# NickQrumpton/lattice-gaussian-mcmc

Measured on AMD Instinct MI355X. Metric: Klein samples/sec at n=512 NTRU (IMHK proposals, d=1024), higher is better.
Workload: dtype f64

## Files before the change

### lattice-gaussian-mcmc_amd/csrc/lgs_capi.hip

```cpp
#include <hip/hip_runtime.h>

#include <algorithm>
#include <cmath>
#include <cstdarg>
#include <cstdio>
#include <cstdlib>
#include <climits>
#include <cstring>
#include <string>
#include <vector>

#include "../../include/lgs.h"
#include "lgs_kernels.h"
#include "lgs_szc_host.h"

namespace {

thread_local std::string g_err;

int fail(int code, const char* fmt, ...) {
    char buf[512];
    va_list ap;
    va_start(ap, fmt);
    vsnprintf(buf, sizeof(buf), fmt, ap);
// ... 109 lines not shown
    bool has_rd = false, oz_off = false;
    DevBuf H16, F0;
    DevBuf ZNZ;
    DevBuf CLIVE;
    DevBuf VNP;
    DevBuf LAGP;
    struct {
        const void* Z = nullptr;
        int64_t lanes = 0, cols = 0;
        const unsigned int* clive = nullptr;
        int64_t clive_ld = 0;
    } hist;
    DevBuf Bd;
    DevBuf kchunk, koff;
    bool bz_mom_ok = false;
    DevBuf MP;
    DevBuf etab;
    DevBuf etab2;
    DevBuf szc;
    bool libm_samplez = false;
    bool has_Bi8 = false;
    int64_t bd_rows = 0, bd_cols = 0;
    std::vector<BzCall> pending_i8;
    bool i8_dev_replay = false;
    DevBuf Z, LW, V, sel, fsel, cnt, ccnt, flags, stage_a, stage_b, stage_c, stage_d, stage_e,
        stage_f, stage_g, stage_h, stage_i, vs;
    int64_t max_props = 1 << 18;
    bool max_props_user = false;
    bool no_pipe = false, no_look = false, no_qskip = false, no_cu_split = false;
    int zint = 2;
    bool timing = false;
    double t_ms[7] = {0, 0, 0, 0, 0, 0, 0};
    int64_t t_n[7] = {0, 0, 0, 0, 0, 0, 0};
    DevBuf dg_x, dg_y, dg_out, dg_a, dg_b, dg_c, dg_t;
    DevBuf DQ, DBIT;
    bool has_q = false, has_binv = false;
    std::vector<Timer> pending;
    std::vector<hipEvent_t> pool;
    unsigned int* fw_host = nullptr;
    hipEvent_t fw_ev = nullptr;
    struct BlockSet {
        DevBuf Z, LW, H16, ZNZ, CLIVE, flags;
        hipEvent_t ev_free = nullptr;
        bool free_recorded = false;
    } bset[3];
    int bset_next = 0;
    int nsets = 2;
    bool kstream_sets_fixed = false;
    hipStream_t kstream = nullptr;
    hipStream_t kstream_full = nullptr, kstream_split = nullptr;
    int cu_split = 0;
    int kstream_cus = 0;
    int split_cus = 0;
    hipEvent_t kt0 = nullptr, kt1 = nullptr;
    bool kt_pending = false;
    double kt_bz_ms = 0.0;
    hipEvent_t ev_klein = nullptr;
    struct Spec {
        bool valid = false;
        uint64_t seed = 0, chain0 = 0, step0 = 0;
        int64_t nc = 0, Tb = 0, ldzb = 0;
        int zb = 0, j = 0;
        bool wl = false, exact = false, oz = false;
        decltype(hist) h;
        hipEvent_t ev = nullptr;
    } spec;
};

// ... 46 lines not shown
struct SetSwap {
    lgs_ctx* c = nullptr;
    int j = -1;
    bool flags_in = false, store_in = false;
    void swap_flags() {
        swap_buf(c->flags, c->bset[j].flags);
        flags_in = !flags_in;
    }
    void swap_store() {
        auto& s = c->bset[j];
        swap_buf(c->Z, s.Z);
        swap_buf(c->LW, s.LW);
        swap_buf(c->H16, s.H16);
        swap_buf(c->ZNZ, s.ZNZ);
        swap_buf(c->CLIVE, s.CLIVE);
        store_in = !store_in;
    }
    void restore() {
        if (j < 0) return;
        if (store_in) swap_store();
        if (flags_in) swap_flags();
    }
    bool record = true;
    void release() {
        if (j < 0) return;
        restore();
        if (record) {
            (void)hipEventRecord(c->bset[j].ev_free, c->stream);
            c->bset[j].free_recorded = true;
        }
        j = -1;
    }
    ~SetSwap() { release(); }
};

constexpr double kBzStoreBytesPerMs = 4.6e9;
static int split_decide(lgs_ctx* c) {
    if (c->cu_split != 0 || !c->kt_pending || hipEventQuery(c->kt1) != hipSuccess) return LGS_OK;
    c->kt_pending = false;
    float ms = 0.f;
    if (hipEventElapsedTime(&ms, c->kt0, c->kt1) != hipSuccess || !(ms > 0.f)) return LGS_OK;
    const int ncu = c->split_cus * 8 / 7;
    const double cost = (double)ms * (double)(ncu - c->split_cus) / (double)c->split_cus;
    if (c->kt_bz_ms > cost) {
        HIP_TRY(hipStreamSynchronize(c->kstream_full));
        c->kstream = c->kstream_split;
        c->kstream_cus = c->split_cus;
        c->cu_split = 1;
    } else {
        c->cu_split = 2;
    }
    return LGS_OK;
}

int spec_discard(lgs_ctx* c) {
    if (!c->spec.valid) return LGS_OK;
    c->spec.valid = false;
    HIP_TRY(hipStreamSynchronize(c->kstream));
    HIP_TRY(hipMemset(c->bset[c->spec.j].flags.p, 0, 4 * lgs::kFlagWords));
    size_t keep = 0;
    for (auto& t : c->pending) {
        if (t.spec) {
            c->pool.push_back(t.a);
            c->pool.push_back(t.b);
        } else {
            c->pending[keep++] = t;
        }
    }
    c->pending.resize(keep);
    return LGS_OK;
}

int settle_bz(lgs_ctx* c, const unsigned int* f0_known = nullptr) {
    if (!f0_known) HIP_TRY(hipStreamSynchronize(c->stream));
    if (c->pending_i8.empty() && !c->i8_dev_replay) return LGS_OK;
    {
        unsigned int f0 = 0;
        if (f0_known)
            f0 = *f0_known;
        else
            HIP_TRY(hipMemcpy(&f0, c->flags.p, sizeof(f0), hipMemcpyDeviceToHost));
// ... 23 lines not shown
        c->z1cap = 2.0 * std::max(z1, c->z1seen);
        c->z1seen = z1;
    }
}

void fold_timers(lgs_ctx* c) {
    size_t keep = 0;
    for (auto& t : c->pending) {
        if (t.spec || hipEventQuery(t.b) != hipSuccess) {
            c->pending[keep++] = t;
            continue;
        }
        float ms = 0;
        if (hipEventElapsedTime(&ms, t.a, t.b) == hipSuccess) {
            c->t_ms[t.kernel] += ms;
            c->t_n[t.kernel] += 1;
        }
        c->pool.push_back(t.a);
        c->pool.push_back(t.b);
    }
    c->pending.resize(keep);
}

int finish(lgs_ctx* c, const unsigned int* fw_known = nullptr, bool clear_all = false) {
    int rc0 = settle_bz(c, fw_known);
    if (rc0) return rc0;
    fold_timers(c);
    unsigned int fw[lgs::kFlagWords] = {};
    if (fw_known)
        memcpy(fw, fw_known, sizeof(fw));
    else
        HIP_TRY(hipMemcpy(fw, c->flags.p, sizeof(fw), hipMemcpyDeviceToHost));
    const unsigned int f = fw[0];
    c->resolved_seen = 0;
    if (fw[1] || fw[2] || fw[3])
        fold_counters(c, fw);
    c->n_accept_resolved += fw[lgs::kFlagWordAcceptResolved];
    c->n_wl_mismatch += fw[lgs::kFlagWordWLMismatch];
    c->n_qskip += fw[lgs::kFlagWordQSkip];
    bool any = false;
    for (int k = 1; k < lgs::kFlagWords; ++k) any |= fw[k] != 0;
    if (clear_all)
        HIP_TRY(hipMemsetAsync(c->flags.p, 0, lgs::kFlagWords * sizeof(unsigned int), c->stream));
    else if (any)
        HIP_TRY(hipMemsetAsync((unsigned int*)c->flags.p + 1, 0, (lgs::kFlagWords - 1) * sizeof(unsigned int),
                               c->stream));
    if (f & lgs::kFlagNonFinite)
        return fail(LGS_ERR_NONFINITE, "non-finite conditional mean (reference raises ValueError)");
    if (f & lgs::kFlagOverflow)
        return fail(LGS_ERR_OVERFLOW, "coefficient |z| >= 2^31: rerun with LGS_Z64");
    return LGS_OK;
}

int finish_or_redo(lgs_ctx* c, bool oz_used, int& zb, bool& redo, bool early = false) {
    redo = false;
    unsigned int fw[lgs::kFlagWords];
    if (early) {
        HIP_TRY(hipEventSynchronize(c->fw_ev));
        memcpy(fw, c->fw_host, sizeof(fw));
    } else {
        HIP_TRY(hipStreamSynchronize(c->stream));
        HIP_TRY(hipMemcpy(fw, c->flags.p, sizeof(fw), hipMemcpyDeviceToHost));
    }
    if (!(fw[0] & lgs::kAbortMask)) return finish(c, fw, early);
    c->pending_i8.clear();
    c->i8_dev_replay = false;
    for (auto& t : c->pending) {
        c->pool.push_back(t.a);
        c->pool.push_back(t.b);
    }
    c->pending.clear();
    c->n_fallback += 1;
    c->n_resolved += fw[kFlagWordCheckpoint];
    if (fw[0] & lgs::kFlagOverflow16) {
        if (zb == 2) c->zint = 4;
        if (oz_used) c->oz_off = true;
    }
    if (fw[0] & lgs::kFlagCarry16) c->zint = 4;
    if (zb == 2) zb = c->zint;
    HIP_TRY(hipMemsetAsync(c->flags.p, 0, 4 * lgs::kFlagWords, c->stream));
    redo = true;
    return LGS_OK;
}

int reset_flags(lgs_ctx* c) {
    int rc = c->flags.reserve(4 * lgs::kFlagWords);
    if (rc) return rc;
    c->resolved_seen = 0;
    HIP_TRY(hipMemsetAsync(c->flags.p, 0, 4 * lgs::kFlagWords, c->stream));
    return LGS_OK;
}

lgs::KleinArgs base_args(lgs_ctx* c, uint64_t seed) {
    lgs::KleinArgs a{};
    const double* co = c->coord.as<double>();
    const int64_t d = c->d;
    a.d = (int)d;
    a.precision = c->precision;
    a.linear_probs = (c->basis_flags & LGS_BASIS_LINEAR_PROBS) ? 1 : 0;
    a.cp = co;
    a.rii = co + d;
    a.sig = co + 2 * d;
    a.sig_ref = co + 3 * d;
// ... 101 lines not shown
    if (zb == 2) {
        c->zint = 4;
        zb = 4;
    }
    if (oz) c->oz_off = true;
    c->hist.Z = nullptr;
    rc = run_klein(c, a, exact, wl, zb, Z, oz);
    if (oz_out) *oz_out = oz;
    return rc;
}

int run_bz_fp64(lgs_ctx* c, const BzCall& b) {
    Scope s(c, 1);
    HIP_TRY(lgs::launch::bz(b.Z, b.zb, b.ldz, b.sel, c->BT.as<double>(), (int)c->d, b.n, b.V, c->d, b.rb,
                            b.rstride, b.roff, c->stream));
    if (b.VN) HIP_TRY(lgs::launch::vnorm2_rows(b.V, (int)c->d, b.vn_n, b.rb, b.rstride, b.roff, b.VN, c->stream));
    return LGS_OK;
}

int run_bz(lgs_ctx* c, const void* Z, int zb, int64_t ldz, int64_t n, double* V,
           int64_t rb = 0, int64_t rstride = 0, int64_t roff = 0, const int64_t* sel = nullptr,
           bool after_klein = false, const unsigned int* abort = nullptr, double* VN = nullptr,
           int64_t vn_n = -1, bool device_replay = false, unsigned long long* MP = nullptr,
           int64_t mp_ld = 0, unsigned int* MPL = nullptr) {
    if (!c->has_B) return fail(LGS_ERR_STATE, "lattice points need B (lgs_set_basis B != NULL)");
    if (vn_n < 0 || vn_n > n) vn_n = n;
    if (vn_n == 0) VN = nullptr;
    BzCall b{Z, zb, ldz, n, V, rb > 0 ? rb : n, rstride, roff, sel, VN, vn_n};
    static const bool force64 = hook_is("LGS_BZ_FP64", 1);
    if (!c->has_Bi8 || force64) {
        Scope s(c, 1);
        HIP_TRY(lgs::launch::bz(b.Z, b.zb, b.ldz, b.sel, c->BT.as<double>(), (int)c->d, b.n, b.V, c->d, b.rb,
                                b.rstride, b.roff, c->stream, abort));
        if (VN) HIP_TRY(lgs::launch::vnorm2_rows(b.V, (int)c->d, vn_n, b.rb, b.rstride, b.roff, VN, c->stream));
        return LGS_OK;
    }
    Scope s(c, 1);
    const int8_t* hi = c->Bd.as<int8_t>();
    const int8_t* lo = hi + (size_t)c->bd_rows * c->bd_cols;
    static const int diag_bz = hook("LGS_DIAG_BZ") ? atoi(hook("LGS_DIAG_BZ")) : 0;
    if (diag_bz & 1) VN = nullptr;
    if (diag_bz & 2) sel = nullptr;
    double* VNP = nullptr;
    if (VN) {
        const int rc = c->VNP.reserve((size_t)2 * ((c->d + lgs::kBzBN - 1) / lgs::kBzBN) * vn_n * 8);
        if (rc) return rc;
        VNP = c->VNP.as<double>();
    }
    HIP_TRY(lgs::launch::bz_i8(Z, zb, ldz, sel, c->kchunk.as<int>(), c->koff.as<int>(), hi, lo,
                               (int)c->bd_cols, (int)c->d, n, V, c->d, b.rb,
                               b.rstride, b.roff, c->flags.as<unsigned int>(),
                               after_klein && c->hist.Z == Z && Z ? c->H16.as<int16_t>() : nullptr, c->hist.lanes,
                               c->hist.cols, c->stream, abort, c->ZNZ.as<uint8_t>(),
                               after_klein && c->hist.Z == Z && Z ? c->hist.clive : nullptr, c->hist.clive_ld,
                               VNP, vn_n, MP, mp_ld, MPL));
    if (VN) HIP_TRY(lgs::launch::vnorm2_reduce(VNP, (int)c->d, vn_n, b.rb, b.rstride, b.roff, VN, c->stream, abort));
    if (device_replay) {
        c->i8_dev_replay = true;
        const unsigned int* need = c->flags.as<unsigned int>();
        HIP_TRY(lgs::launch::bz(b.Z, b.zb, b.ldz, b.sel, c->BT.as<double>(), (int)c->d, b.n, b.V, c->d, b.rb,
                                b.rstride, b.roff, c->stream, abort, need));
        if (VN)
            HIP_TRY(lgs::launch::vnorm2_rows(b.V, (int)c->d, vn_n, b.rb, b.rstride, b.roff, VN, c->stream, abort,
                                             need));
        return LGS_OK;
    }
    c->pending_i8.push_back(b);
    return LGS_OK;
}

int lookahead(lgs_ctx* c, int j, uint64_t seed, uint64_t first_chain, uint64_t step0, int64_t nc, int64_t tb,
              bool carry, int zb, bool exact, bool wl) {
    const auto hist = c->hist;
    SetSwap sw;
    sw.c = c;
    sw.j = j;
    sw.record = false;
    sw.swap_flags();
    sw.swap_store();
    const int64_t ldz = nc * tb + (carry ? nc : 0);
    lgs::KleinArgs a = base_args(c, seed);
    a.counter_mode = 1;
    a.chain0 = (uint32_t)first_chain;
    a.step0 = (uint32_t)step0;
    a.nt = tb;
    a.n = nc * tb;
    a.ldz = ldz;
    a.LW = c->LW.as<double>();
    auto& bs = c->bset[j];
    if (bs.free_recorded) HIP_TRY(hipStreamWaitEvent(c->kstream, bs.ev_free, 0));
// ... 796 lines not shown
        }
        if ((rc = spec_discard(c))) return rc;
        for (int si = 0; si < c->nsets; ++si) {
            auto& s = c->bset[si];
            s.Z.release();
            s.LW.release();
            s.H16.release();
            s.ZNZ.release();
            s.CLIVE.release();
        }
        c->Z.release();
        c->LW.release();
        c->cnt.release();
        c->LWE.release();
        c->H16.release();
        c->ZNZ.release();
        c->CLIVE.release();
        c->hist = decltype(c->hist){};
        maxp = std::max<int64_t>(nc * thin, maxp / 2);
        c->max_props = maxp;
        c->max_props_user = true;
    }
    const bool no_look = c->no_look || hook_is("LGS_NO_LOOKAHEAD", 1);
    bool spec_hit = false;
    if (c->spec.valid) {
        const int64_t tb0 = std::min<int64_t>(T, n_steps);
        const auto& sp = c->spec;
        spec_hit = pipe && sp.seed == seed && sp.chain0 == first_chain && sp.step0 == first_step && sp.nc == nc &&
                   sp.Tb == tb0 && sp.ldzb == nc * tb0 + (carry ? nc : 0) && sp.zb == zb && sp.wl == wl &&
                   sp.exact == exact && sp.j == c->bset_next;
        if (!spec_hit && (rc = spec_discard(c))) return rc;
    }

    void* zs = z_state;
    double* lws = logw_state;
    int32_t* init = state_init;
    int64_t* acc = accepts;
    if (!dev) {
        if ((rc = c->stage_a.reserve((size_t)nc * d * ob)) || (rc = c->stage_b.reserve((size_t)nc * 8)) ||
            (rc = c->stage_c.reserve((size_t)nc * 4)) || (rc = c->stage_d.reserve((size_t)nc * 8)))
            return rc;
        zs = c->stage_a.p;
        lws = c->stage_b.as<double>();
        init = c->stage_c.as<int32_t>();
        acc = c->stage_d.as<int64_t>();
        HIP_TRY(hipMemcpyAsync(zs, z_state, (size_t)nc * d * ob, hipMemcpyHostToDevice, c->stream));
        HIP_TRY(hipMemcpyAsync(lws, logw_state, nc * 8, hipMemcpyHostToDevice, c->stream));
        HIP_TRY(hipMemcpyAsync(init, state_init, nc * 4, hipMemcpyHostToDevice, c->stream));
        HIP_TRY(hipMemcpyAsync(acc, accepts, nc * 8, hipMemcpyHostToDevice, c->stream));
    }
    double* lwk = logw_samples;
    uint8_t* accs = accepted;
    if (!dev && (logw_samples || accepted)) {
        if ((rc = c->stage_h.reserve((size_t)std::max<int64_t>(nc * n_keep, 1) * 8)) ||
            (rc = c->stage_i.reserve((size_t)std::max<int64_t>(nc * n_steps, 1))))
            return rc;
        lwk = logw_samples ? c->stage_h.as<double>() : nullptr;
        accs = accepted ? (uint8_t*)c->stage_i.p : nullptr;
    }
    unsigned long long* mom = nullptr;
    if (moments) {
        if (dev) {
            mom = (unsigned long long*)moments;
        } else {
            if ((rc = c->stage_e.reserve((size_t)2 * d * 8))) return rc;
            mom = c->stage_e.as<unsigned long long>();
            HIP_TRY(hipMemcpyAsync(mom, moments, (size_t)2 * d * 8, hipMemcpyHostToDevice, c->stream));
        }
    }
    unsigned int* fl = c->flags.as<unsigned int>();

    const uint64_t next_step = first_step + (uint64_t)n_steps;
    bool look_done = false;
    static const bool look_late = !hook_is("LGS_LOOKAHEAD_EARLY", 1);
    for (int64_t t0 = 0; t0 < n_steps || t0 == 0;) {
        bool oz_used = false;
        SetSwap sw;
        if (pipe) {
            sw.c = c;
            sw.j = c->bset_next;
            sw.swap_flags();
            fl = c->flags.as<unsigned int>();
        }
        if (t0 == 0) {
            HIP_TRY(lgs::launch::uninit_scan(init, nc, fl + kFlagWordUninit, c->stream));
            lgs::KleinArgs a = base_args(c, seed);
            a.counter_mode = 1;
            a.chain0 = (uint32_t)first_chain;
            a.step0 = 0;
            a.nt = 1;
            a.n = nc;
            a.ldz = nc;
            a.LW = c->LW.as<double>();
            if (certw) a.emax = c->EMAX.as<unsigned long long>();
            a.gate = fl + kFlagWordUninit;
            bool oz0 = false;
            if ((rc = run_klein_store(c, a, exact, wl, zb, c->Z.p, true, &oz0))) return rc;
            oz_used |= oz0;
            HIP_TRY(lgs::launch::init_apply(c->Z.p, zb, init, nc, (int)d, c->LW.as<double>(), zs, ob, cm, lws,
// ... 4 lines not shown
            if ((rc = finish_or_redo(c, oz_used, zb, redo))) return rc;
            if (redo) continue;
            break;
        }
        const int64_t Tb = std::min<int64_t>(T, n_steps - t0);
        const int64_t npb = nc * Tb;
        const int64_t first_keep = t0 / thin;
        const int64_t kb = std::min<int64_t>(Tb / thin, n_keep - first_keep);
        if (pipe) sw.swap_store();
        lgs::KleinArgs a = base_args(c, seed);
        a.counter_mode = 1;
        a.chain0 = (uint32_t)first_chain;
        a.step0 = (uint32_t)(first_step + (uint64_t)t0);
        const int64_t ldzb = npb + (carry ? nc : 0);
        a.nt = Tb;
        a.n = npb;
        a.ldz = ldzb;
        a.LW = c->LW.as<double>();
        if (certw) {
            a.LWE = c->LWE.as<double>();
            a.emax = c->EMAX.as<unsigned long long>();
        }
        bool ozb = false;
        if (pipe && spec_hit && t0 == 0) {
            spec_hit = false;
            c->spec.valid = false;
            for (auto& t : c->pending) t.spec = false;
            ozb = c->spec.oz;
            c->hist = c->spec.h;
            HIP_TRY(hipStreamWaitEvent(c->stream, c->spec.ev, 0));
        } else if (pipe) {
            auto& bs = c->bset[sw.j];
            if (bs.free_recorded) HIP_TRY(hipStreamWaitEvent(c->kstream, bs.ev_free, 0));
            const hipStream_t cs = c->stream;
            const bool timed = c->cu_split == 0 && !c->kt_pending;
            if (timed) HIP_TRY(hipEventRecord(c->kt0, c->kstream));
            c->stream = c->kstream;
            rc = run_klein_store(c, a, exact, wl, zb, c->Z.p, true, &ozb);
            c->stream = cs;
            if (rc) return rc;
            if (timed) {
                HIP_TRY(hipEventRecord(c->kt1, c->kstream));
                c->kt_pending = true;
                c->kt_bz_ms = carry ? (double)nc * (double)kb * 8.0 * (double)d / kBzStoreBytesPerMs : 0.0;
            }
            HIP_TRY(hipEventRecord(c->ev_klein, c->kstream));
            HIP_TRY(hipStreamWaitEvent(c->stream, c->ev_klein, 0));
        } else if ((rc = run_klein_store(c, a, exact, wl, zb, c->Z.p, true, &ozb))) {
            return rc;
        }
        if (pipe && !no_look && !look_late && !look_done && t0 + T >= n_steps &&
            next_step + (uint64_t)n_steps <= (1ull << 32)) {
            look_done = true;
            if ((rc = lookahead(c, (sw.j + 1) % c->nsets, seed, first_chain, next_step, nc, std::min<int64_t>(T, n_steps), carry,
                                zb, exact, wl)))
                return rc;
        }
        oz_used |= ozb;
        if (carry && kb > 0)
            HIP_TRY(lgs::launch::carry_cols(zs, ob, cm, nc, (int)d, c->Z.p, zb, ldzb, npb, c->stream, fl));
        if (early) {
            HIP_TRY(hipMemcpyAsync(c->fw_host, fl, 4 * lgs::kFlagWords, hipMemcpyDeviceToHost, c->stream));
            HIP_TRY(hipEventRecord(c->fw_ev, c->stream));
        }
        if (moments) HIP_TRY(hipMemsetAsync(c->cnt.p, 0, (size_t)npb * 4, c->stream));
        lgs::AcceptArgs aa{};
        aa.nc = nc;
        aa.T = Tb;
        aa.thin = thin;
        aa.n_keep = std::max<int64_t>(kb, 1);
        aa.seed = seed;
        aa.chain0 = (uint32_t)first_chain;
        aa.step0 = a.step0;
        aa.LW = c->LW.as<double>();
        aa.lw_state = lws;
        aa.accepts = acc;
        aa.sel = (z_samples || v_samples || zk_samples) && kb > 0 ? c->sel.as<int64_t>() : nullptr;
        aa.final_sel = c->fsel.as<int64_t>();
        aa.carry_col = carry ? npb : -1;
// ... 21 lines not shown
            aa.bscale = bs ? std::max(1.0, atof(bs)) : 1.0;
        }
        {
            Scope s(c, 2);
            HIP_TRY(lgs::launch::accept(aa, a, c->stream));
        }
        static const bool no_bz_mom = hook_is("LGS_NO_BZ_MOMENTS", 1);
        static const bool bz_f64 = hook_is("LGS_BZ_FP64", 1);
        const bool bz_mom = moments && v_samples && early && thin == 1 && kb == Tb && kb > 0 && zb == 2 &&
                            c->has_Bi8 && c->bz_mom_ok && !bz_f64 && c->hist.Z == c->Z.p && c->hist.Z &&
                            c->hist.clive != nullptr && lgs::launch::bz_moments_supported() &&
                            d % 16 == 0 && d <= lgs::kOzMaxD && npb < ((int64_t)1 << 32) && !no_bz_mom;
        const bool fuse_final = !bz_mom && moments && !((z_samples || zk_samples) && kb > 0 && !carry) &&
                                npb < ((int64_t)1 << 32);
        if (moments && !bz_mom) {
            Scope s(c, 3);
            HIP_TRY(lgs::launch::moments_carry(zs, ob, cm, nc, (int)d, c->ccnt.as<int32_t>(), mom, c->stream, fl));
            const bool zflags = c->hist.Z == c->Z.p && c->hist.Z != nullptr;
            HIP_TRY(lgs::launch::moments_final(c->Z.p, zb, ldzb, c->cnt.as<int32_t>(), npb, Tb,
                                               fuse_final ? c->fsel.as<int64_t>() : nullptr, (int)d, mom, zs,
                                               ob, cm, nc, c->stream, fl, zflags ? c->ZNZ.as<uint8_t>() : nullptr,
                                               c->hist.lanes, (int)((16 - d % 16) % 16)));
        }
        if ((z_samples || v_samples || zk_samples) && kb > 0) {
            const int64_t nq = nc * kb;
            if (v_samples) {
                const bool dev_replay = early || (lag && lag->lag_v_sums && vnorm2_samples);
                const int64_t ntiles = (nq + 63) / 64, mp_ld = c->bd_cols;
                const int64_t ngw = (d + 2047) / 2048;
                unsigned int* mpl = nullptr;
                if (bz_mom) {
                    if ((rc = c->MP.reserve((size_t)ntiles * (mp_ld * 8 + ngw * 4)))) return rc;
                    mpl = (unsigned int*)(c->MP.as<unsigned long long>() + (size_t)ntiles * mp_ld);
                }
                if ((rc = run_bz(c, c->Z.p, zb, ldzb, nq, v_samples, kb, n_keep, first_keep,
                                 c->sel.as<int64_t>(), true, fl, vnorm2_samples, fn_chains * kb, dev_replay,
                                 bz_mom ? c->MP.as<unsigned long long>() : nullptr, mp_ld, mpl)))
                    return rc;
                if (bz_mom) {
                    Scope s(c, 3);
                    HIP_TRY(lgs::launch::bz_moments_reduce(c->MP.as<unsigned long long>(), mpl, ntiles, mp_ld,
                                                           (int)d, mom, fl, c->stream, fl));
                    HIP_TRY(lgs::launch::moments_carry(zs, ob, cm, nc, (int)d, c->ccnt.as<int32_t>(), mom,
                                                       c->stream, fl, fl));
                    HIP_TRY(lgs::launch::moments_final(c->Z.p, zb, ldzb, c->cnt.as<int32_t>(), npb, Tb, nullptr,
                                                       (int)d, mom, zs, ob, cm, nc, c->stream, fl,
                                                       c->ZNZ.as<uint8_t>(), c->hist.lanes, 0, fl));
                }
            }
            if (zk_samples)
                HIP_TRY(lgs::launch::coord_gather(c->Z.p, zb, ldzb, c->sel.as<int64_t>(), fn_chains * kb, kb, zs, ob, cm, nc,
                                                  (int)d, (int)zk_index, zk_samples, kb, n_keep, first_keep,
                                                  c->stream, fl));
            if (lag) {
                const int L = (int)lag->lag_L;
                if ((rc = c->LAGP.reserve((size_t)(L + 2) * fn_chains * 8))) return rc;
                if (lag->lag_z_sums)
                    HIP_TRY(lgs::launch::lag_update(zk_samples + first_keep, 0, n_keep, fn_chains, kb, L, 1.0,
                                                    lag->lag_z_ring, lag->lag_z_sums, c->LAGP.p, c->stream, fl));
                if (lag->lag_v_sums)
                    HIP_TRY(lgs::launch::lag_update(vnorm2_samples + first_keep, 1, n_keep, fn_chains, kb, L,
                                                    lag->lag_v_scale, lag->lag_v_ring, lag->lag_v_sums, c->LAGP.p,
                                                    c->stream, fl));
            }
            if (z_samples) {
                if ((rc = c->stage_f.reserve((size_t)nq * d * ob))) return rc;
                HIP_TRY(lgs::launch::gather_z(c->Z.p, zb, ldzb, c->sel.as<int64_t>(), nq, kb, zs, ob, cm,
                                              nc, (int)d, c->stage_f.p, 1, c->stream, fl));
                if ((rc = c->stage_g.reserve((size_t)nq * d * ob))) return rc;
                HIP_TRY(lgs::launch::transpose_out(c->stage_f.p, ob, nq, nq, (int)d, c->stage_g.p,
                                                   ob, c->stream));
                HIP_TRY(hipMemcpy2DAsync((char*)z_samples + (size_t)first_keep * d * ob,
                                         (size_t)n_keep * d * ob, c->stage_g.p, (size_t)kb * d * ob,
                                         (size_t)kb * d * ob, nc, kind_of(dev, true), c->stream));
            }
        }
        if (bz_mom)
            HIP_TRY(lgs::launch::final_h16(c->H16.as<int16_t>(), c->hist.lanes, c->fsel.as<int64_t>(), nc, (int)d,
                                           zs, ob, cm, c->stream, fl));
        else if (!fuse_final)
            HIP_TRY(lgs::launch::gather_z(c->Z.p, zb, ldzb, c->fsel.as<int64_t>(), nc, 1, zs, ob, cm, nc,
                                          (int)d, zs, cm, c->stream, fl));
        bool redo = false;
        if ((rc = finish_or_redo(c, oz_used, zb, redo, early))) return rc;
        if (pipe) {
            sw.release();
            fl = c->flags.as<unsigned int>();
            if (!redo) c->bset_next = (c->bset_next + 1) % c->nsets;
        }
        if (redo) continue;
        t0 += T;
    }
    if (pipe && (rc = split_decide(c))) return rc;
    if (pipe && !no_look && look_late && next_step + (uint64_t)n_steps <= (1ull << 32))
        if ((rc = lookahead(c, c->bset_next, seed, first_chain, next_step, nc, std::min<int64_t>(T, n_steps), carry, zb,
                            exact, wl)))
            return rc;
    if (!dev) {
        HIP_TRY(hipMemcpyAsync(z_state, zs, (size_t)nc * d * ob, hipMemcpyDeviceToHost, c->stream));
        HIP_TRY(hipMemcpyAsync(logw_state, lws, nc * 8, hipMemcpyDeviceToHost, c->stream));
        HIP_TRY(hipMemcpyAsync(state_init, init, nc * 4, hipMemcpyDeviceToHost, c->stream));
        HIP_TRY(hipMemcpyAsync(accepts, acc, nc * 8, hipMemcpyDeviceToHost, c->stream));
        if (moments)
            HIP_TRY(hipMemcpyAsync(moments, mom, (size_t)2 * d * 8, hipMemcpyDeviceToHost, c->stream));
        if (logw_samples && n_keep > 0)
            HIP_TRY(hipMemcpyAsync(logw_samples, lwk, (size_t)nc * n_keep * 8, hipMemcpyDeviceToHost, c->stream));
        if (accepted && n_steps > 0)
            HIP_TRY(hipMemcpyAsync(accepted, accs, (size_t)nc * n_steps, hipMemcpyDeviceToHost, c->stream));
        HIP_TRY(hipStreamSynchronize(c->stream));
    }
    return LGS_OK;
}

int lgs_sample_z(lgs_ctx* c, int64_t n, const double* mu, const double* sigma, const double* u,
                 int32_t precision, int64_t* z_out, double* log_norm_out, uint32_t flags) {
    int rc = check_ctx(c, false);
    if (rc) return rc;
// ... 536 lines not shown
```

### lattice-gaussian-mcmc_amd/csrc/lgs_kernels.h

```cpp
#pragma once
#include <hip/hip_runtime.h>
#include <stdint.h>

#ifndef LGS_R6_OFF
#ifndef LGS_REC_L2
#define LGS_REC_L2 1
#endif
#ifndef LGS_REC_NOPIN
#define LGS_REC_NOPIN 1
#endif
#ifndef LGS_PHILOX_HOIST
#define LGS_PHILOX_HOIST 1
#endif
#endif

namespace lgs {

constexpr unsigned int kFlagNonFinite = 1u;
constexpr unsigned int kFlagOverflow = 2u;
constexpr unsigned int kFlagI8Range = 4u;
constexpr unsigned int kFlagOverflow16 = 8u;
constexpr unsigned int kFlagCarry16 = 16u;
constexpr unsigned int kAbortMask = kFlagOverflow16 | kFlagCarry16;
constexpr int kFlagWordResolved = 1;
// ... 187 lines not shown
hipError_t klein(const KleinArgs& a, const double* R, const double* RP, const double* RC,
                 int panel, int kernel, bool wl, int zb, void* Z, hipStream_t st);
hipError_t accept(const AcceptArgs& a, const KleinArgs& ka, hipStream_t st);
hipError_t samplez_probe(const double* mu, const double* sig, const double* u, int64_t n,
                         int precision, int linear, int mode, const double* etab, int64_t* z, double* ln,
                         hipStream_t st);
hipError_t log_density(const KleinArgs& a, const double* R, const void* Z, int zb, double* out,
                       hipStream_t st);
hipError_t moments_final(const void* Z, int zb, int64_t ldz, const int32_t* cnt, int64_t n, int64_t T,
                         const int64_t* fsel, int d, unsigned long long* mom, void* zs, int ob,
                         int zs_cm, int64_t nc, hipStream_t st, const unsigned int* abort,
                         const uint8_t* znz = nullptr, int64_t zlanes = 0, int zshift = 0,
                         const unsigned int* need = nullptr);
hipError_t moments_carry(const void* zs, int zb, int coord_major, int64_t nc, int d,
                         const int32_t* cc, unsigned long long* mom, hipStream_t st,
                         const unsigned int* abort = nullptr, const unsigned int* need = nullptr);
hipError_t gather_z(const void* Z, int zb, int64_t ldz, const int64_t* sel, int64_t nq,
                    int64_t q_per_chain, const void* zs, int ob, int zs_coord_major, int64_t nc,
                    int d, void* out, int out_coord_major, hipStream_t st,
                    const unsigned int* abort = nullptr);
hipError_t uninit_scan(const int32_t* init, int64_t nc, unsigned int* any, hipStream_t st);
hipError_t init_apply(const void* Z, int zb, int32_t* init, int64_t nc, int d, const double* LW, void* zs,
                      int ob, int zs_cm, double* lws, unsigned int* flags, hipStream_t st);
hipError_t transpose_out(const void* Z, int zb, int64_t ldz, int64_t n, int d, void* out, int ob,
                         hipStream_t st);
hipError_t to_coord_major(const void* in, int ib, int64_t n, int d, void* Z, int zb, int64_t ldz,
                          hipStream_t st);
hipError_t bz(const void* Z, int zb, int64_t ldz, const int64_t* sel, const double* BT, int d,
              int64_t n, double* V, int64_t ldv, int64_t rb, int64_t rstride, int64_t roff,
              hipStream_t st, const unsigned int* abort = nullptr, const unsigned int* need = nullptr);
hipError_t bz_i8(const void* Z, int zb, int64_t ldz, const int64_t* sel, const int* kchunk,
                 const int* koff, const int8_t* Bd1, const int8_t* Bd0, int dc, int d, int64_t n,
                 double* V, int64_t ldv, int64_t rb, int64_t rstride, int64_t roff,
                 unsigned int* flags, const int16_t* h16, int64_t h16_lanes, int64_t hcols,
                 hipStream_t st, const unsigned int* abort = nullptr, const uint8_t* znz = nullptr,
                 const unsigned int* clive = nullptr, int64_t clive_ld = 0, double* VNP = nullptr,
                 int64_t vn_n = 0, unsigned long long* MP = nullptr, int64_t mp_ld = 0,
                 unsigned int* MPL = nullptr);
hipError_t bz_moments_reduce(const unsigned long long* MP, const unsigned int* MPL, int64_t ntiles, int64_t mp_ld,
                             int d,
                             unsigned long long* mom, const unsigned int* flags, hipStream_t st,
                             const unsigned int* abort);
hipError_t final_h16(const int16_t* h16, int64_t lanes, const int64_t* fsel, int64_t nc, int d, void* zs,
                     int ob, int zs_cm, hipStream_t st, const unsigned int* abort);
hipError_t vnorm2_reduce(const double* VNP, int d, int64_t n, int64_t rb, int64_t rstride, int64_t roff,
                         double* VN, hipStream_t st, const unsigned int* abort = nullptr);
// ... 20 lines not shown
```

### lattice-gaussian-mcmc_amd/csrc/lgs_kernels.hip

```cpp
#include <hip/hip_runtime.h>

#include <type_traits>
#include <stdint.h>

#if !defined(LGS_NEAR_UNROLLED) && !defined(LGS_CAPPED_CALL) && !defined(LGS_CAPPED_INLINE)
#define LGS_CAPPED_INLINE
#endif
#include "lgs_device.h"
#include "lgs_kernels.h"

namespace lgs {

typedef unsigned int v4u_t __attribute__((ext_vector_type(4)));

__device__ __forceinline__ void lane_counter(const KleinArgs& a, int64_t p, uint32_t& chain,
                                             uint32_t& step) {
    if (a.counter_mode == 0) {
        const uint64_t s = a.base + (uint64_t)p;
        chain = (uint32_t)s;
        step = (uint32_t)(s >> 32);
    } else {
        chain = a.chain0 + (uint32_t)(p / a.nt);
        step = a.step0 + (uint32_t)(p % a.nt);
    }
// ... 2325 lines not shown
    if (out) atomicOr(flags, kFlagOverflow16);
}

template <typename OT, typename ZT>
__global__ __launch_bounds__(256) void carry_cols_kernel(const OT* __restrict__ zs, int zs_coord_major,
                                                         int64_t nc, int d, ZT* __restrict__ Z,
                                                         int64_t ldz, int64_t col0, unsigned int* flags) {
    const int64_t c = (int64_t)blockIdx.x * blockDim.x + threadIdx.x;
    const int i = blockIdx.y;
    if (c >= nc) return;
    const OT v = zs_coord_major ? zs[(size_t)i * nc + c] : zs[(size_t)c * d + i];
    if (sizeof(ZT) == 2 && flags && (v > (OT)32767 || v < (OT)-32768)) atomicOr(flags, kFlagCarry16);
    Z[(size_t)i * ldz + col0 + c] = (ZT)v;
}

__global__ __launch_bounds__(256) void uninit_scan_kernel(const int32_t* __restrict__ init, int64_t nc,
                                                          unsigned int* any) {
    bool u = false;
    for (int64_t c = (int64_t)blockIdx.x * blockDim.x + threadIdx.x; c < nc; c += (int64_t)gridDim.x * blockDim.x)
        u |= init[c] == 0;
    if (__builtin_amdgcn_ballot_w64(u) != 0 && (threadIdx.x & 63) == 0) atomicOr(any, 1u);
}

template <typename ZT, typename OT>
__global__ __launch_bounds__(256) void init_apply_kernel(const ZT* __restrict__ Z, int32_t* __restrict__ init,
                                                         int64_t nc, int d, const double* __restrict__ LW,
                                                         OT* __restrict__ zs, int zs_cm, double* __restrict__ lws,
                                                         unsigned int* flags) {
    const bool ab = aborted(flags);
    if (blockIdx.x == 0 && threadIdx.x == 0) flags[kFlagWordCheckpoint] = ab ? 0u : flags[kFlagWordResolved];
    if (flags[kFlagWordUninit] == 0u || ab) return;
    const int64_t c = (int64_t)blockIdx.x * blockDim.x + threadIdx.x;
    if (c >= nc || init[c] != 0) return;
    for (int i = 0; i < d; ++i) {
        const OT v = (OT)Z[(size_t)i * nc + c];
        if (zs_cm)
            zs[(size_t)i * nc + c] = v;
        else
            zs[(size_t)c * d + i] = v;
    }
    lws[c] = LW[c];
    init[c] = kInitStep0;
}

template <typename ZT, typename OT>
__global__ __launch_bounds__(256) void transpose_kernel(const ZT* __restrict__ Z, int64_t ldz,
// ... 792 lines not shown
    if (n <= 0) return hipSuccess;
    const int nparts = 2 * ((d + kBzBN - 1) / kBzBN);
    hipLaunchKernelGGL(vnorm2_reduce_kernel, dim3((unsigned)((n + 255) / 256)), dim3(256), 0, st, VNP, nparts, n, rb,
                       rstride, roff, VN, abort);
    return hipGetLastError();
}

hipError_t vnorm2_rows(const double* V, int d, int64_t n, int64_t rb, int64_t rstride, int64_t roff, double* VN,
                       hipStream_t st, const unsigned int* abort, const unsigned int* need) {
    if (n <= 0) return hipSuccess;
    const int64_t nb = (n + 3) / 4;
    hipLaunchKernelGGL(vnorm2_rows_kernel, dim3((unsigned)(need ? std::min<int64_t>(nb, 16) : nb)), dim3(256), 0, st,
                       V, d, n, rb, rstride, roff, VN, abort, need);
    return hipGetLastError();
}

hipError_t uninit_scan(const int32_t* init, int64_t nc, unsigned int* any, hipStream_t st) {
    if (nc <= 0) return hipSuccess;
    const unsigned g = (unsigned)std::min<int64_t>((nc + 255) / 256, 1024);
    hipLaunchKernelGGL(uninit_scan_kernel, dim3(g), dim3(256), 0, st, init, nc, any);
    return hipGetLastError();
}

hipError_t init_apply(const void* Z, int zb, int32_t* init, int64_t nc, int d, const double* LW, void* zs,
                      int ob, int zs_cm, double* lws, unsigned int* flags, hipStream_t st) {
    if (nc <= 0) return hipSuccess;
    const dim3 grid((unsigned)((nc + 255) / 256));
    LGS_ZT(zb, ZT, LGS_ZT(ob, OT, hipLaunchKernelGGL((init_apply_kernel<ZT, OT>), grid, dim3(256), 0, st, (const ZT*)Z, init, nc, d, LW, (OT*)zs, zs_cm, lws, flags)));
    return hipGetLastError();
}

hipError_t check_range16(const void* zs, int ob, int64_t count, unsigned int* flags, hipStream_t st) {
    if (count <= 0) return hipSuccess;
    const dim3 grid((unsigned)std::min<int64_t>((count + 255) / 256, 2048));
    LGS_ZT(ob, OT, hipLaunchKernelGGL(range16_kernel<OT>, grid, dim3(256), 0, st, (const OT*)zs, count, flags));
    return hipGetLastError();
}

hipError_t carry_cols(const void* zs, int ob, int zs_coord_major, int64_t nc, int d, void* Z, int zb,
                      int64_t ldz, int64_t col0, hipStream_t st, unsigned int* flags) {
    if (nc <= 0) return hipSuccess;
    const dim3 grid((unsigned)((nc + 255) / 256), (unsigned)d);
    LGS_ZT(ob, OT, LGS_ZT(zb, ZT, hipLaunchKernelGGL((carry_cols_kernel<OT, ZT>), grid, dim3(256), 0, st, (const OT*)zs, zs_coord_major, nc, d, (ZT*)Z, ldz, col0, flags)));
    return hipGetLastError();
}

// ... 140 lines not shown
```

Before: 124.9 million.

## Overlap per-block lookahead Klein with deferred vnorm, moments and lag reductions

Speculative lookahead now runs after every step block, not only the last one, so the next block's Klein sampling on the side stream can overlap the current block's tail work. A flags-handover kernel snapshots and clears the flag words early. That lets the block set be released and the tail reductions (vnorm2, bz moments, lag updates) run against the snapshot while the next lookahead proceeds. spec_discard now waits on the spec event instead of synchronizing the whole stream. The cost is added complexity in redo and abort handling, with a risk of wasted speculative work when blocks are redone.

Result: no change. 125.2 million (median of 6 runs) (+0.2%).

```diff
diff --git a/lattice-gaussian-mcmc_amd/csrc/lgs_capi.hip b/lattice-gaussian-mcmc_amd/csrc/lgs_capi.hip
--- a/lattice-gaussian-mcmc_amd/csrc/lgs_capi.hip
+++ b/lattice-gaussian-mcmc_amd/csrc/lgs_capi.hip
@@ -155,6 +155,8 @@
     bool has_Bi8 = false;
     int64_t bd_rows = 0, bd_cols = 0;
     std::vector<BzCall> pending_i8;
+    BzCall vn_later;
+    bool has_vn_later = false;
     bool i8_dev_replay = false;
     DevBuf Z, LW, V, sel, fsel, cnt, ccnt, flags, stage_a, stage_b, stage_c, stage_d, stage_e,
         stage_f, stage_g, stage_h, stage_i, vs;
@@ -177,6 +179,7 @@
         hipEvent_t ev_free = nullptr;
         bool free_recorded = false;
     } bset[3];
+    DevBuf flsnap;
     int bset_next = 0;
     int nsets = 2;
     bool kstream_sets_fixed = false;
@@ -269,13 +272,16 @@
         if (flags_in) swap_flags();
     }
     bool record = true;
+    void record_free() {
+        if (j < 0 || !record) return;
+        (void)hipEventRecord(c->bset[j].ev_free, c->stream);
+        c->bset[j].free_recorded = true;
+        record = false;
+    }
     void release() {
         if (j < 0) return;
         restore();
-        if (record) {
-            (void)hipEventRecord(c->bset[j].ev_free, c->stream);
-            c->bset[j].free_recorded = true;
-        }
+        record_free();
         j = -1;
     }
     ~SetSwap() { release(); }
@@ -303,7 +309,7 @@
 int spec_discard(lgs_ctx* c) {
     if (!c->spec.valid) return LGS_OK;
     c->spec.valid = false;
-    HIP_TRY(hipStreamSynchronize(c->kstream));
+    HIP_TRY(hipEventSynchronize(c->spec.ev));
     HIP_TRY(hipMemset(c->bset[c->spec.j].flags.p, 0, 4 * lgs::kFlagWords));
     size_t keep = 0;
     for (auto& t : c->pending) {
@@ -373,7 +379,7 @@
     c->pending.resize(keep);
 }
 
-int finish(lgs_ctx* c, const unsigned int* fw_known = nullptr, bool clear_all = false) {
+int finish(lgs_ctx* c, const unsigned int* fw_known = nullptr, bool clear_all = false, bool cleared = false) {
     int rc0 = settle_bz(c, fw_known);
     if (rc0) return rc0;
     fold_timers(c);
@@ -391,7 +397,9 @@
     c->n_qskip += fw[lgs::kFlagWordQSkip];
     bool any = false;
     for (int k = 1; k < lgs::kFlagWords; ++k) any |= fw[k] != 0;
-    if (clear_all)
+    if (cleared)
+        ;
+    else if (clear_all)
         HIP_TRY(hipMemsetAsync(c->flags.p, 0, lgs::kFlagWords * sizeof(unsigned int), c->stream));
     else if (any)
         HIP_TRY(hipMemsetAsync((unsigned int*)c->flags.p + 1, 0, (lgs::kFlagWords - 1) * sizeof(unsigned int),
@@ -403,7 +411,7 @@
     return LGS_OK;
 }
 
-int finish_or_redo(lgs_ctx* c, bool oz_used, int& zb, bool& redo, bool early = false) {
+int finish_or_redo(lgs_ctx* c, bool oz_used, int& zb, bool& redo, bool early = false, bool cleared = false) {
     redo = false;
     unsigned int fw[lgs::kFlagWords];
     if (early) {
@@ -413,14 +421,19 @@
         HIP_TRY(hipStreamSynchronize(c->stream));
         HIP_TRY(hipMemcpy(fw, c->flags.p, sizeof(fw), hipMemcpyDeviceToHost));
     }
-    if (!(fw[0] & lgs::kAbortMask)) return finish(c, fw, early);
+    if (!(fw[0] & lgs::kAbortMask)) return finish(c, fw, early, cleared);
     c->pending_i8.clear();
     c->i8_dev_replay = false;
+    size_t keep = 0;
     for (auto& t : c->pending) {
+        if (t.spec) {
+            c->pending[keep++] = t;
+            continue;
+        }
         c->pool.push_back(t.a);
         c->pool.push_back(t.b);
     }
-    c->pending.clear();
+    c->pending.resize(keep);
     c->n_fallback += 1;
     c->n_resolved += fw[kFlagWordCheckpoint];
     if (fw[0] & lgs::kFlagOverflow16) {
@@ -429,7 +442,7 @@
     }
     if (fw[0] & lgs::kFlagCarry16) c->zint = 4;
     if (zb == 2) zb = c->zint;
-    HIP_TRY(hipMemsetAsync(c->flags.p, 0, 4 * lgs::kFlagWords, c->stream));
+    if (!cleared) HIP_TRY(hipMemsetAsync(c->flags.p, 0, 4 * lgs::kFlagWords, c->stream));
     redo = true;
     return LGS_OK;
 }
@@ -577,7 +590,7 @@
            int64_t rb = 0, int64_t rstride = 0, int64_t roff = 0, const int64_t* sel = nullptr,
            bool after_klein = false, const unsigned int* abort = nullptr, double* VN = nullptr,
            int64_t vn_n = -1, bool device_replay = false, unsigned long long* MP = nullptr,
-           int64_t mp_ld = 0, unsigned int* MPL = nullptr) {
+           int64_t mp_ld = 0, unsigned int* MPL = nullptr, bool vn_later = false) {
     if (!c->has_B) return fail(LGS_ERR_STATE, "lattice points need B (lgs_set_basis B != NULL)");
     if (vn_n < 0 || vn_n > n) vn_n = n;
     if (vn_n == 0) VN = nullptr;
@@ -609,18 +622,35 @@
                                c->hist.cols, c->stream, abort, c->ZNZ.as<uint8_t>(),
                                after_klein && c->hist.Z == Z && Z ? c->hist.clive : nullptr, c->hist.clive_ld,
                                VNP, vn_n, MP, mp_ld, MPL));
-    if (VN) HIP_TRY(lgs::launch::vnorm2_reduce(VNP, (int)c->d, vn_n, b.rb, b.rstride, b.roff, VN, c->stream, abort));
+    vn_later = vn_later && device_replay && VN;
+    if (VN && !vn_later)
+        HIP_TRY(lgs::launch::vnorm2_reduce(VNP, (int)c->d, vn_n, b.rb, b.rstride, b.roff, VN, c->stream, abort));
     if (device_replay) {
         c->i8_dev_replay = true;
         const unsigned int* need = c->flags.as<unsigned int>();
         HIP_TRY(lgs::launch::bz(b.Z, b.zb, b.ldz, b.sel, c->BT.as<double>(), (int)c->d, b.n, b.V, c->d, b.rb,
                                 b.rstride, b.roff, c->stream, abort, need));
-        if (VN)
+        if (vn_later) {
+            b.VN = VN;
+            b.vn_n = vn_n;
+            c->vn_later = b;
+            c->has_vn_later = true;
+        } else if (VN)
             HIP_TRY(lgs::launch::vnorm2_rows(b.V, (int)c->d, vn_n, b.rb, b.rstride, b.roff, VN, c->stream, abort,
                                              need));
         return LGS_OK;
     }
     c->pending_i8.push_back(b);
+    return LGS_OK;
+}
+
+int run_bz_vn(lgs_ctx* c, const unsigned int* fw) {
+    if (!c->has_vn_later) return LGS_OK;
+    c->has_vn_later = false;
+    const BzCall& b = c->vn_later;
+    HIP_TRY(lgs::launch::vnorm2_reduce(c->VNP.as<double>(), (int)c->d, b.vn_n, b.rb, b.rstride, b.roff, b.VN, c->stream,
+                                       fw));
+    HIP_TRY(lgs::launch::vnorm2_rows(b.V, (int)c->d, b.vn_n, b.rb, b.rstride, b.roff, b.VN, c->stream, fw, fw));
     return LGS_OK;
 }
 
@@ -1463,15 +1493,13 @@
         c->max_props_user = true;
     }
     const bool no_look = c->no_look || hook_is("LGS_NO_LOOKAHEAD", 1);
-    bool spec_hit = false;
-    if (c->spec.valid) {
-        const int64_t tb0 = std::min<int64_t>(T, n_steps);
+    auto spec_matches = [&](uint64_t step0, int64_t tb) {
         const auto& sp = c->spec;
-        spec_hit = pipe && sp.seed == seed && sp.chain0 == first_chain && sp.step0 == first_step && sp.nc == nc &&
-                   sp.Tb == tb0 && sp.ldzb == nc * tb0 + (carry ? nc : 0) && sp.zb == zb && sp.wl == wl &&
-                   sp.exact == exact && sp.j == c->bset_next;
-        if (!spec_hit && (rc = spec_discard(c))) return rc;
-    }
+        return pipe && sp.valid && sp.seed == seed && sp.chain0 == first_chain && sp.step0 == step0 && sp.nc == nc &&
+               sp.Tb == tb && sp.ldzb == nc * tb + (carry ? nc : 0) && sp.zb == zb && sp.wl == wl &&
+               sp.exact == exact && sp.j == c->bset_next;
+    };
+    if (c->spec.valid && !spec_matches(first_step, std::min<int64_t>(T, n_steps)) && (rc = spec_discard(c))) return rc;
 
     void* zs = z_state;
     double* lws = logw_state;
@@ -1512,10 +1540,15 @@
     unsigned int* fl = c->flags.as<unsigned int>();
 
     const uint64_t next_step = first_step + (uint64_t)n_steps;
-    bool look_done = false;
-    static const bool look_late = !hook_is("LGS_LOOKAHEAD_EARLY", 1);
+    const bool look_next_call = !no_look && next_step + (uint64_t)n_steps <= (1ull << 32);
+    const bool look_late = hook_is("LGS_LOOKAHEAD_LATE", 1);
+    if (pipe && (rc = c->flsnap.reserve(4 * lgs::kFlagWords))) return rc;
     for (int64_t t0 = 0; t0 < n_steps || t0 == 0;) {
         bool oz_used = false;
+        c->has_vn_later = false;
+        if (pipe && c->spec.valid && !spec_matches(first_step + (uint64_t)t0, std::min<int64_t>(T, n_steps - t0)) &&
+            (rc = spec_discard(c)))
+            return rc;
         SetSwap sw;
         if (pipe) {
             sw.c = c;
@@ -1566,8 +1599,7 @@
             a.emax = c->EMAX.as<unsigned long long>();
         }
         bool ozb = false;
-        if (pipe && spec_hit && t0 == 0) {
-            spec_hit = false;
+        if (pipe && c->spec.valid) {
             c->spec.valid = false;
             for (auto& t : c->pending) t.spec = false;
             ozb = c->spec.oz;
@@ -1592,13 +1624,6 @@
             HIP_TRY(hipStreamWaitEvent(c->stream, c->ev_klein, 0));
         } else if ((rc = run_klein_store(c, a, exact, wl, zb, c->Z.p, true, &ozb))) {
             return rc;
-        }
-        if (pipe && !no_look && !look_late && !look_done && t0 + T >= n_steps &&
-            next_step + (uint64_t)n_steps <= (1ull << 32)) {
-            look_done = true;
-            if ((rc = lookahead(c, (sw.j + 1) % c->nsets, seed, first_chain, next_step, nc, std::min<int64_t>(T, n_steps), carry,
-                                zb, exact, wl)))
-                return rc;
         }
         oz_used |= ozb;
         if (carry && kb > 0)
@@ -1666,46 +1691,33 @@
                                                ob, cm, nc, c->stream, fl, zflags ? c->ZNZ.as<uint8_t>() : nullptr,
                                                c->hist.lanes, (int)((16 - d % 16) % 16)));
         }
+        const int64_t ntiles = (nc * kb + 63) / 64, mp_ld = c->bd_cols;
+        unsigned int* mpl = nullptr;
         if ((z_samples || v_samples || zk_samples) && kb > 0) {
             const int64_t nq = nc * kb;
+            if (zk_samples)
+                HIP_TRY(lgs::launch::coord_gather(c->Z.p, zb, ldzb, c->sel.as<int64_t>(), fn_chains * kb, kb, zs, ob, cm, nc,
+                                                  (int)d, (int)zk_index, zk_samples, kb, n_keep, first_keep,
+                                                  c->stream, fl));
             if (v_samples) {
                 const bool dev_replay = early || (lag && lag->lag_v_sums && vnorm2_samples);
-                const int64_t ntiles = (nq + 63) / 64, mp_ld = c->bd_cols;
                 const int64_t ngw = (d + 2047) / 2048;
-                unsigned int* mpl = nullptr;
                 if (bz_mom) {
                     if ((rc = c->MP.reserve((size_t)ntiles * (mp_ld * 8 + ngw * 4)))) return rc;
                     mpl = (unsigned int*)(c->MP.as<unsigned long long>() + (size_t)ntiles * mp_ld);
                 }
                 if ((rc = run_bz(c, c->Z.p, zb, ldzb, nq, v_samples, kb, n_keep, first_keep,
                                  c->sel.as<int64_t>(), true, fl, vnorm2_samples, fn_chains * kb, dev_replay,
-                                 bz_mom ? c->MP.as<unsigned long long>() : nullptr, mp_ld, mpl)))
+                                 bz_mom ? c->MP.as<unsigned long long>() : nullptr, mp_ld, mpl, pipe)))
                     return rc;
                 if (bz_mom) {
                     Scope s(c, 3);
-                    HIP_TRY(lgs::launch::bz_moments_reduce(c->MP.as<unsigned long long>(), mpl, ntiles, mp_ld,
-                                                           (int)d, mom, fl, c->stream, fl));
                     HIP_TRY(lgs::launch::moments_carry(zs, ob, cm, nc, (int)d, c->ccnt.as<int32_t>(), mom,
                                                        c->stream, fl, fl));
                     HIP_TRY(lgs::launch::moments_final(c->Z.p, zb, ldzb, c->cnt.as<int32_t>(), npb, Tb, nullptr,
                                                        (int)d, mom, zs, ob, cm, nc, c->stream, fl,
                                                        c->ZNZ.as<uint8_t>(), c->hist.lanes, 0, fl));
                 }
-            }
-            if (zk_samples)
-                HIP_TRY(lgs::launch::coord_gather(c->Z.p, zb, ldzb, c->sel.as<int64_t>(), fn_chains * kb, kb, zs, ob, cm, nc,
-                                                  (int)d, (int)zk_index, zk_samples, kb, n_keep, first_keep,
-                                                  c->stream, fl));
-            if (lag) {
-                const int L = (int)lag->lag_L;
-                if ((rc = c->LAGP.reserve((size_t)(L + 2) * fn_chains * 8))) return rc;
-                if (lag->lag_z_sums)
-                    HIP_TRY(lgs::launch::lag_update(zk_samples + first_keep, 0, n_keep, fn_chains, kb, L, 1.0,
-                                                    lag->lag_z_ring, lag->lag_z_sums, c->LAGP.p, c->stream, fl));
-                if (lag->lag_v_sums)
-                    HIP_TRY(lgs::launch::lag_update(vnorm2_samples + first_keep, 1, n_keep, fn_chains, kb, L,
-                                                    lag->lag_v_scale, lag->lag_v_ring, lag->lag_v_sums, c->LAGP.p,
-                                                    c->stream, fl));
             }
             if (z_samples) {
                 if ((rc = c->stage_f.reserve((size_t)nq * d * ob))) return rc;
@@ -1725,18 +1737,53 @@
         else if (!fuse_final)
             HIP_TRY(lgs::launch::gather_z(c->Z.p, zb, ldzb, c->fsel.as<int64_t>(), nc, 1, zs, ob, cm, nc,
                                           (int)d, zs, cm, c->stream, fl));
+        const unsigned int* fl_late = fl;
+        if (pipe) {
+            HIP_TRY(lgs::launch::flags_handover(fl, c->flsnap.as<unsigned int>(), c->stream));
+            sw.record_free();
+            fl_late = c->flsnap.as<unsigned int>();
+        }
+        if ((rc = run_bz_vn(c, fl_late))) return rc;
+        if (bz_mom && v_samples) {
+            Scope s(c, 3);
+            HIP_TRY(lgs::launch::bz_moments_reduce(c->MP.as<unsigned long long>(), mpl, ntiles, mp_ld, (int)d, mom,
+                                                   fl_late, c->stream, fl_late));
+        }
+        if (lag && (z_samples || v_samples || zk_samples) && kb > 0) {
+            const int L = (int)lag->lag_L;
+            if ((rc = c->LAGP.reserve((size_t)(L + 2) * fn_chains * 8))) return rc;
+            if (lag->lag_z_sums)
+                HIP_TRY(lgs::launch::lag_update(zk_samples + first_keep, 0, n_keep, fn_chains, kb, L, 1.0,
+                                                lag->lag_z_ring, lag->lag_z_sums, c->LAGP.p, c->stream, fl_late));
+            if (lag->lag_v_sums)
+                HIP_TRY(lgs::launch::lag_update(vnorm2_samples + first_keep, 1, n_keep, fn_chains, kb, L,
+                                                lag->lag_v_scale, lag->lag_v_ring, lag->lag_v_sums, c->LAGP.p,
+                                                c->stream, fl_late));
+        }
+        if (pipe && !look_late) {
+            const int64_t t1 = t0 + T;
+            const int jn = (sw.j + 1) % c->nsets;
+            if (t1 < n_steps)
+                rc = lookahead(c, jn, seed, first_chain, first_step + (uint64_t)t1, nc, std::min<int64_t>(T, n_steps - t1),
+                               carry, zb, exact, wl);
+            else if (look_next_call)
+                rc = lookahead(c, jn, seed, first_chain, next_step, nc, std::min<int64_t>(T, n_steps), carry, zb, exact,
+                               wl);
+            if (rc) return rc;
+        }
         bool redo = false;
-        if ((rc = finish_or_redo(c, oz_used, zb, redo, early))) return rc;
+        if ((rc = finish_or_redo(c, oz_used, zb, redo, early, pipe))) return rc;
         if (pipe) {
             sw.release();
             fl = c->flags.as<unsigned int>();
             if (!redo) c->bset_next = (c->bset_next + 1) % c->nsets;
+            if (redo && (rc = spec_discard(c))) return rc;
         }
         if (redo) continue;
         t0 += T;
     }
     if (pipe && (rc = split_decide(c))) return rc;
-    if (pipe && !no_look && look_late && next_step + (uint64_t)n_steps <= (1ull << 32))
+    if (pipe && look_next_call && look_late)
         if ((rc = lookahead(c, c->bset_next, seed, first_chain, next_step, nc, std::min<int64_t>(T, n_steps), carry, zb,
                             exact, wl)))
             return rc;
diff --git a/lattice-gaussian-mcmc_amd/csrc/lgs_kernels.h b/lattice-gaussian-mcmc_amd/csrc/lgs_kernels.h
--- a/lattice-gaussian-mcmc_amd/csrc/lgs_kernels.h
+++ b/lattice-gaussian-mcmc_amd/csrc/lgs_kernels.h
@@ -233,6 +233,7 @@
 hipError_t uninit_scan(const int32_t* init, int64_t nc, unsigned int* any, hipStream_t st);
 hipError_t init_apply(const void* Z, int zb, int32_t* init, int64_t nc, int d, const double* LW, void* zs,
                       int ob, int zs_cm, double* lws, unsigned int* flags, hipStream_t st);
+hipError_t flags_handover(unsigned int* flags, unsigned int* snap, hipStream_t st);
 hipError_t transpose_out(const void* Z, int zb, int64_t ldz, int64_t n, int d, void* out, int ob,
                          hipStream_t st);
 hipError_t to_coord_major(const void* in, int ib, int64_t n, int d, void* Z, int zb, int64_t ldz,
diff --git a/lattice-gaussian-mcmc_amd/csrc/lgs_kernels.hip b/lattice-gaussian-mcmc_amd/csrc/lgs_kernels.hip
--- a/lattice-gaussian-mcmc_amd/csrc/lgs_kernels.hip
+++ b/lattice-gaussian-mcmc_amd/csrc/lgs_kernels.hip
@@ -2371,6 +2371,14 @@
     if (__builtin_amdgcn_ballot_w64(u) != 0 && (threadIdx.x & 63) == 0) atomicOr(any, 1u);
 }
 
+__global__ __launch_bounds__(64) void flags_handover_kernel(unsigned int* __restrict__ flags,
+                                                            unsigned int* __restrict__ snap) {
+    const int i = threadIdx.x;
+    if (i >= kFlagWords) return;
+    snap[i] = flags[i];
+    flags[i] = 0u;
+}
+
 template <typename ZT, typename OT>
 __global__ __launch_bounds__(256) void init_apply_kernel(const ZT* __restrict__ Z, int32_t* __restrict__ init,
                                                          int64_t nc, int d, const double* __restrict__ LW,
@@ -3209,6 +3217,11 @@
     return hipGetLastError();
 }
 
+hipError_t flags_handover(unsigned int* flags, unsigned int* snap, hipStream_t st) {
+    hipLaunchKernelGGL(flags_handover_kernel, dim3(1), dim3(64), 0, st, flags, snap);
+    return hipGetLastError();
+}
+
 hipError_t init_apply(const void* Z, int zb, int32_t* init, int64_t nc, int d, const double* LW, void* zs,
                       int ob, int zs_cm, double* lws, unsigned int* flags, hipStream_t st) {
     if (nc <= 0) return hipSuccess;
```
